# mschoenb97/po2_quantization

Hardware: AMD Instinct MI355X
Metric: quantized-conv fwd images/sec, ResNet56 224×224 bs=256; 1/2/4/8 MI355X (higher is better)
Workload: dtype fp32(bf16x3); 1 GPU; resnet56 quantized-conv chain: 56 fused po2-4bit quantize+conv fwd + head (stage-1 and stage-2 conv1->conv2 pairs as one launch each) (stride-2 conv1 + 1x1 shortcut of stages 2-3 as one launch each) (weight packs of the single-conv layers batched: one launch per 36); conv_pairs=True, conv_pairs_stage2=True, s2ds=True, pack_batch=True, autotune=True, image=224, batch_per_gpu=256, global_batch=256, quantizer=po2, bits=4, precision=bf16x3, parallelism=dp1, world_size=1, hip_graph=False

## Files before the change

### po2_quantization_amd/csrc/po2q_conv_pair64.hip

```cpp
#include <hip/hip_runtime.h>

#include <algorithm>
#include <climits>
#include <cstdint>
#include <cstdlib>
#include <map>
#include <mutex>
#include <string>
#include <type_traits>
#include <utility>

#include "../../include/po2q.h"
#include "po2q_internal.h"
#include "po2q_rows_dev.h"
#include "po2q_x3_dev.h"

namespace po2q {

namespace {
constexpr int kP6C = 64;
constexpr int kP6Wp = 64;
constexpr int kP6PL = (kP6Wp + 2) * 2 * kP6C;
constexpr int kP6Set = 3 * kP6PL;
constexpr int kP6Raw = kP6C * kP6Wp * 4;
constexpr int kP6RPB = kP6Wp * 4;
constexpr int kP6PD = 2;
constexpr int kP6KS = 6;
constexpr int kP6Lds = kP6PD * kP6Raw + 2 * kP6Set + 2 * kP6Set;
constexpr int kP6PackBytes = 3 * kP6KS * 4 * 64 * 16;

__device__ __forceinline__ int p6_addr(int P, int oc) { return P * 128 + ((oc ^ (P & 7)) << 4); }
}

struct Pair64Args {
    int N, H, W;
    int RB, nseg, items, remap;
    const uint4* wp1;
    const uint4* wp2;
    const float* s1;
    const float* s2;
    const float* b1;
    const float* b2;
};

template <int NG, int NTS>
__global__ __launch_bounds__(512, 1) void conv_pair64(const float* __restrict__ x, float* __restrict__ y,
                                                      Pair64Args a) {
    static_assert(NG == 3 || NG == 4, "column groups");
    constexpr int C = kP6C, KS = kP6KS, PL = kP6PL, SET = kP6Set, RPB = kP6RPB;
    extern __shared__ __attribute__((aligned(16))) unsigned char lds[];
    const int tid = threadIdx.x, lane = tid & 63;
    const int wave = __builtin_amdgcn_readfirstlane(tid >> 6);
    const bool roleA = wave >= 4;
    const int t = wave & 3;
    unsigned char* raw = lds;
    unsigned char* xp = raw + kP6PD * kP6Raw;

    int blk = blockIdx.x;
    if (a.remap) blk = (blk & 7) * (int)(gridDim.x >> 3) + (blk >> 3);
    if (blk >= a.items) return;
    const int seg = blk % a.nseg;
    const int n = blk / a.nseg;
    const int p0 = seg * a.RB;
    const int rbe = min(a.RB, a.H - p0);
    const int nx = rbe + 4;
    const int n1 = rbe + 2;
    const int nsteps = nx + 2;
    const int HW = a.H * a.W;
// ... 10 lines not shown
    float bk[4];
    {
        const float* b = roleA ? a.b2 : a.b1;
#pragma unroll
        for (int e = 0; e < 4; ++e) bk[e] = b ? b[roleA ? 16 * t + (lane & 15) : 16 * t + 4 * (lane >> 4) + e] : 0.0f;
    }
#pragma unroll
    for (int r = 0; r < 3; ++r)
#pragma unroll
        for (int ks = 0; ks < KS; ++ks) asm volatile("s_waitcnt vmcnt(0)" : "+v"(bw[r][ks]));
    asm volatile("s_waitcnt vmcnt(0)" : "+v"(scale), "+v"(bk[0]), "+v"(bk[1]), "+v"(bk[2]), "+v"(bk[3]));

    for (int e = tid; e < (4 * SET) / 16; e += 512) reinterpret_cast<uint4*>(xp)[e] = make_uint4(0u, 0u, 0u, 0u);
    __syncthreads();

    const __amdgpu_buffer_rsrc_t rs = rows_rsrc(x + (int64_t)n * C * HW, C * HW * 4);
    uint32_t vi[4];
#pragma unroll
    for (int i = 0; i < 4; ++i) {
        const int c = 16 * t + 4 * i + (lane >> 4), q = 4 * (lane & 15);
        vi[i] = q < a.W ? ((uint32_t)c * (uint32_t)HW + (uint32_t)q) * 4u : 0x7fffffffu;
    }
    const uint32_t raw_lds = (uint32_t)(uintptr_t)raw;
    auto load_x = [&](int sl, int jn) __attribute__((always_inline)) {
        const int h = p0 - 2 + jn;
        const bool hok = jn < nx && h >= 0 && h < a.H;
        const uint32_t roff = (uint32_t)(hok ? h : 0) * (uint32_t)a.W * 4u;
        const uint32_t base = raw_lds + (uint32_t)(sl * kP6Raw) + (uint32_t)(16 * t) * (uint32_t)RPB;
#pragma unroll
        for (int i = 0; i < 4; ++i)
            rows_dma16<(NTS & 2) != 0>(rs, (hok && vi[i] != 0x7fffffffu) ? vi[i] + roff : 0x7fffffffu, 0u,
                                       base + (uint32_t)i * 1024u);
    };
    int xwb[2] = {p6_addr(lane + 1, 2 * t) + kP6PD * kP6Raw, p6_addr(lane + 1, 2 * t + 1) + kP6PD * kP6Raw};
    asm volatile("" : "+v"(xwb[0]), "+v"(xwb[1]));
    auto split_x = [&](const unsigned char* rw, int pb) __attribute__((always_inline)) {
#pragma unroll
        for (int o = 0; o < 2; ++o) {
            uint32_t b8[8];
#pragma unroll
            for (int e = 0; e < 8; ++e)
                b8[e] = *reinterpret_cast<const uint32_t*>(rw + (16 * t + 8 * o + e) * RPB + lane * 4);
            uint4 hi, mid, lo;
            split3(b8, hi, mid, lo);
            unsigned char* pw = lds + (xwb[o] + pb);
            *reinterpret_cast<uint4*>(pw) = hi;
            *reinterpret_cast<uint4*>(pw + PL) = mid;
            *reinterpret_cast<uint4*>(pw + 2 * PL) = lo;
        }
    };

    int foff[KS];
    {
        const int p = lane & 15, g = lane >> 4;
        const int region = kP6PD * kP6Raw + (roleA ? 2 * SET : 0);
#pragma unroll
        for (int ks = 0; ks < KS; ++ks) {
            foff[ks] = p6_addr(p + ks % 3, 4 * (ks / 3) + g) + region;
            asm volatile("" : "+v"(foff[ks]));
        }
    }
    int ywb = p6_addr((lane & 15) + 1, 2 * t + (lane >> 5)) + 8 * ((lane >> 4) & 1) + kP6PD * kP6Raw + 2 * SET;
    asm volatile("" : "+v"(ywb));

    floatx4 acc[3][NG];
#pragma unroll
    for (int sl = 0; sl < 3; ++sl)
#pragma unroll
        for (int grp = 0; grp < NG; ++grp) acc[sl][grp] = floatx4{0.f, 0.f, 0.f, 0.f};

    auto mfmas = [&](auto S_, auto TR_, int pb) __attribute__((always_inline)) {
// ... 3 lines not shown
        bf16x8 af[2][NG];
        auto ldf = [&](bf16x8 (&f)[NG], int st) __attribute__((always_inline)) {
#pragma unroll
            for (int grp = 0; grp < NG; ++grp)
                f[grp] = __builtin_bit_cast(
                    bf16x8, *reinterpret_cast<const uint4*>(lds + (foff[st / 3] + (pb + (st % 3) * PL + grp * (16 * 128)))));
        };
        ldf(af[0], 0);
#pragma unroll
        for (int st = 0; st < 3 * KS; ++st) {
            if (st + 1 < 3 * KS) ldf(af[(st + 1) & 1], st + 1);
            const int ks = st / 3;
#pragma unroll
            for (int rr = 0; rr < 3; ++rr)
#pragma unroll
                for (int grp = 0; grp < NG; ++grp)
                    acc[SL[rr]][grp] =
                        TR ? __builtin_amdgcn_mfma_f32_16x16x32_bf16(bw[rr][ks], af[st & 1][grp], acc[SL[rr]][grp], 0, 0, 0)
                           : __builtin_amdgcn_mfma_f32_16x16x32_bf16(af[st & 1][grp], bw[rr][ks], acc[SL[rr]][grp], 0, 0, 0);
            __builtin_amdgcn_sched_barrier(0);
        }
    };

    floatx4 pend[NG];
#pragma unroll
    for (int grp = 0; grp < NG; ++grp) pend[grp] = floatx4{0.f, 0.f, 0.f, 0.f};

    auto stepB = [&](auto S_, int j) __attribute__((always_inline)) {
        constexpr int S6 = decltype(S_)::value;
        constexpr int S = S6 % 3;
        constexpr int D = (S + 2) % 3;
        constexpr int B2 = S6 & 1;
        asm volatile("s_waitcnt lgkmcnt(0)\n\ts_barrier" ::: "memory");
        load_x(B2, j + 2);
        {
            const int i1 = j - 3;
            const int r1 = p0 - 1 + i1;
            const bool irow = i1 >= 0 && i1 < n1 && r1 >= 0 && r1 < a.H;
            const int p = lane & 15;
            unsigned char* yw = lds + (ywb + (1 - B2) * SET);
#pragma unroll
            for (int grp = 0; grp < NG; ++grp) {
                const int q = 16 * grp + p;
                const bool okq = irow && q < a.W;
                uint32_t b4[4];
#pragma unroll
                for (int e = 0; e < 4; ++e) {
                    const float v = pend[grp][e] * scale + bk[e];
                    b4[e] = okq ? __float_as_uint(v) : 0u;
                }
                uint2 h2, m2, l2;
                split4p(b4, h2, m2, l2);
                unsigned char* yg = yw + grp * (16 * 128);
                *reinterpret_cast<uint2*>(yg) = h2;
                *reinterpret_cast<uint2*>(yg + PL) = m2;
                *reinterpret_cast<uint2*>(yg + 2 * PL) = l2;
            }
        }
        rows_wait<4>();
        split_x(raw + (1 - B2) * kP6Raw, (1 - B2) * SET);
        {
            const int h = p0 - 2 + j;
            if (j < nx && h >= 0 && h < a.H) mfmas(std::integral_constant<int, S>{}, std::true_type{}, B2 * SET);
        }
#pragma unroll
        for (int grp = 0; grp < NG; ++grp) {
            pend[grp] = acc[D][grp];
            acc[D][grp] = floatx4{0.f, 0.f, 0.f, 0.f};
        }
    };

    const __amdgpu_buffer_rsrc_t ry = rows_rsrc(y + (int64_t)n * C * HW, C * HW * 4);

    auto stepA = [&](auto S_, int j) __attribute__((always_inline)) {
        constexpr int S6 = decltype(S_)::value;
        constexpr int S = S6 % 3;
        constexpr int D = (S + 2) % 3;
        constexpr int YR = S6 & 1;
        asm volatile("s_waitcnt lgkmcnt(0)\n\ts_barrier" ::: "memory");
        {
            const int i2 = j - 4, r2 = p0 - 1 + i2;
            if (i2 >= 0 && i2 < n1 && r2 >= 0 && r2 < a.H)
                mfmas(std::integral_constant<int, S>{}, std::false_type{}, YR * SET);
        }
        const int o = j - 6;
        const bool orow = o >= 0 && o < rbe;
// ... 71 lines not shown

hipError_t pair64_launch(const float* x, float* y, int64_t N, int64_t H, int64_t W, const uint16_t* packed1,
                         const float* scale1, const uint16_t* packed2, const float* scale2, const float* bias1,
                         const float* bias2, hipStream_t s) {
    if (!pair64_geom_ok(N, kP6C, H, W)) return hipErrorInvalidValue;
    int64_t nseg = std::max<int64_t>(1, (256 + N - 1) / N);
    nseg = std::min<int64_t>(nseg, std::max<int64_t>(1, H / 8));
    if (const char* e = getenv("PO2Q_PAIR64_NSEG")) nseg = std::min<int64_t>(std::max(1, atoi(e)), H);
    Pair64Args a;
    a.N = (int)N; a.H = (int)H; a.W = (int)W;
    a.RB = (int)((H + nseg - 1) / nseg);
    a.nseg = (int)((H + a.RB - 1) / a.RB);
    const int64_t items = N * a.nseg;
    if (items > INT_MAX / 2) return hipErrorInvalidValue;
    const int blocks = (int)((items + 7) / 8 * 8);
    a.items = (int)items;
    a.remap = 1;
    a.wp1 = reinterpret_cast<const uint4*>(packed1);
    a.wp2 = reinterpret_cast<const uint4*>(packed2);
    a.s1 = scale1; a.s2 = scale2;
    a.b1 = bias1; a.b2 = bias2;
    int nts = 0;
    if (const char* e = getenv("PO2Q_PAIR64_NTS")) nts = atoi(e) == 0 ? 0 : 3;
    const dim3 grid((unsigned)blocks), block(512);
#define PO2Q_P6(g, t)                                                                            \
    if ((W <= 48 ? 3 : 4) == g && nts == t) {                                                    \
        hipLaunchKernelGGL((conv_pair64<g, t>), grid, block, (size_t)kP6Lds, s, x, y, a);        \
        return hipGetLastError();                                                                \
    }
    PO2Q_P6(4, 3) PO2Q_P6(3, 3) PO2Q_P6(4, 0) PO2Q_P6(3, 0)
#undef PO2Q_P6
    return hipErrorInvalidValue;
}

ConvPlan pair64_pack_plan(int64_t N, int64_t H, int64_t W) {
    ConvPlan p{};
    p.N = (int)N; p.C = kP6C; p.H = (int)H; p.W = (int)W; p.K = kP6C;
    p.R = p.S = 3; p.sh = p.sw = 1; p.ph = p.pw = 1; p.dh = p.dw = 1; p.groups = 1;
    p.P = p.H; p.Q = p.W; p.Cg = p.C; p.Kg = p.K;
    p.kind = KIND_BF16X3_ROWS;
    p.vrx = 1;
    p.CC = 32;
    p.nchunks = 2;
    p.steps = kP6KS;
    p.NT = 4;
    p.taps = 9;
    p.packed_floats = kP6PackBytes / 4;
    return p;
}

namespace {
constexpr size_t kP6Scratch = 256 + 2 * ((kP6PackBytes + 255) / 256 * 256);
char* pair64_scratch(hipStream_t s) {
// ... 77 lines not shown
```

### po2_quantization_amd/csrc/po2q_conv_pairw.hip

```cpp
#include <hip/hip_runtime.h>

#include <algorithm>
#include <climits>
#include <cstdint>
#include <cstdlib>
#include <string>
#include <type_traits>
#include <utility>

#include "../../include/po2q.h"
#include "po2q_epi.h"
#include "po2q_internal.h"
#include "po2q_quant_dev.h"
#include "po2q_rows_dev.h"
#include "po2q_x3_dev.h"

namespace po2q {

namespace {
constexpr int kPWC = 32;
constexpr int kPWSW = 32;
constexpr int kPWWaves = 4;
constexpr int kPWWp = kPWSW * kPWWaves;
constexpr int kPWPL = (kPWSW + 2) * 2 * kPWC + 32;
// ... 4 lines not shown

__device__ __forceinline__ int pw_oct(int P, int oc) { return P * 64 + 16 * (oc ^ ((P >> 1) & 3)); }

template <class F, int... R>
__device__ __forceinline__ void pw_unroll(F& f, std::integer_sequence<int, R...>) {
    (f(std::integral_constant<int, R>{}), ...);
}
}

struct PairWArgs {
    int N, H, W;
    int RB, nseg, items, remap;
    WQuant q1, q2;
    const float* b1;
    const float* b2;
    const float* ps1;
    const float* pb1;
    const float* ps2;
    const float* pb2;
    int act1, act2;
    const float* res;
};

template <int PD, int NTS, bool RES, int E, int DBG = 0>
__global__ __launch_bounds__(512, 1) void conv_pairw(const float* __restrict__ x, float* __restrict__ y,
                                                     PairWArgs a) {
    static_assert(PD >= 2 && PD <= 5, "raw ring slots");
    constexpr int CC = kPWC, SW = kPWSW, WC = SW + 2, PL = kPWPL, YPL = kPWYPL, RPB = kPWRPB;
    constexpr int NG = SW / 16, NT = CC / 16, KS = 3, NF = 3 * KS * NT;
    constexpr int yslot = 3 * YPL;
    extern __shared__ __attribute__((aligned(16))) unsigned char lds[];
    const int tid = threadIdx.x, lane = tid & 63;
    const int wave = __builtin_amdgcn_readfirstlane(tid >> 6);
    const bool roleA = wave >= kPWWaves;
    const int sw = wave & (kPWWaves - 1);
    unsigned char* raw = lds;
    unsigned char* yr = raw + PD * kPWRaw;
    unsigned char* slab = yr + 2 * yslot + sw * (3 * PL);
    unsigned char* resr = yr + 2 * yslot + kPWWaves * 3 * PL + sw * (PD * kPWRes);

    int blk = blockIdx.x;
    if (a.remap) blk = (blk & 7) * (int)(gridDim.x >> 3) + (blk >> 3);
    if (blk >= a.items) return;
    const int seg = blk % a.nseg;
    const int n = blk / a.nseg;
    const int p0 = seg * a.RB;
    const int rbe = min(a.RB, a.H - p0);
    const int nx = rbe + 4;
    const int n1 = rbe + 2;
    const int nsteps = nx + 2;
    const int q0 = sw * SW;
    const int HW = a.H * a.W;

    const __amdgpu_buffer_rsrc_t rs = rows_rsrc(x + (int64_t)n * CC * HW, CC * HW * 4);
    uint32_t vi[4];
#pragma unroll
    for (int i = 0; i < 4; ++i) {
        const int e = 64 * (4 * sw + i) + lane;
        const int c = e >> 5, q = 4 * (e & 31);
        vi[i] = q < a.W ? ((uint32_t)c * (uint32_t)HW + (uint32_t)q) * 4u : 0x7fffffffu;
    }
    const uint32_t raw_lds = (uint32_t)(uintptr_t)raw;
// ... 26 lines not shown
                              res_lds + (uint32_t)(sl * kPWRes) + i * 1024u);
    };

    const int cp = lane & 15, so = lane >> 4;
    const int rdx0 = (so * 8) * RPB + (q0 + 2 * cp) * 4;
    const int wa0 = pw_oct(2 * cp + 1, so), wa1 = pw_oct(2 * cp + 2, so);
    const int hl = lane & 31;
    const int hside = hl >> 4, hch = 16 * (lane >> 5) + (hl & 15);
    const int hq = hside ? q0 + SW : q0 - 1;
    const bool h_ok = hq >= 0 && hq < a.W;
    const int wa_h = pw_oct(hside ? WC - 1 : 0, hch >> 3) + (hch & 7) * 2;
    const int rdx_h = hch * RPB + (h_ok ? hq : 0) * 4;
    int foff[NG][KS];
    {
        const int p = lane & 15, g = lane >> 4;
#pragma unroll
        for (int grp = 0; grp < NG; ++grp)
#pragma unroll
            for (int ks = 0; ks < KS; ++ks) foff[grp][ks] = pw_oct((roleA ? q0 : 0) + 16 * grp + p + ks, g);
    }

    const __amdgpu_buffer_rsrc_t ry = rows_rsrc(y + (int64_t)n * CC * HW, CC * HW * 4);
    constexpr int ST = 2 * NT;
    constexpr int VMW_B = 4 * (PD - 2);
    constexpr int VMW_A = ST + (PD - 2) * (4 + ST);

    float scale = 1.0f;
    bool fin = true;
    bf16x8 bw[NF] = {};
    float bk[E ? NT * 4 : 1], es[E ? NT * 4 : 1], eb[E ? NT * 4 : 1];
    floatx4 acc[3][NG][NT];
#pragma unroll
    for (int sl = 0; sl < 3; ++sl)
#pragma unroll
        for (int grp = 0; grp < NG; ++grp)
#pragma unroll
            for (int nt = 0; nt < NT; ++nt) acc[sl][grp][nt] = floatx4{0.f, 0.f, 0.f, 0.f};

    auto mfmas = [&](auto S_, auto TR_, const unsigned char* pb) __attribute__((always_inline)) {
        constexpr int SR = decltype(S_)::value;
        constexpr bool TR = decltype(TR_)::value;
        constexpr int SL[3] = {(SR + 1) % 3, SR, (SR + 2) % 3};
        constexpr int PLS = TR ? PL : YPL;
        bf16x8 af[3][NG];
#pragma unroll
        for (int pl = 0; pl < 3; ++pl)
#pragma unroll
// ... 15 lines not shown
                        acc[SL[rr]][grp][nt] = TR ? __builtin_amdgcn_mfma_f32_16x16x32_bf16(b, af[pl][grp], c, 0, 0, 0)
                                                  : __builtin_amdgcn_mfma_f32_16x16x32_bf16(af[pl][grp], b, c, 0, 0, 0);
                    }
                    if (ks + 1 < KS)
                        af[pl][grp] = __builtin_bit_cast(
                            bf16x8, *reinterpret_cast<const uint4*>(pb + pl * PLS + foff[grp][ks + 1 < KS ? ks + 1 : 0]));
                }
    };

    auto zero_slot = [&](auto S_) __attribute__((always_inline)) {
        constexpr int SR = decltype(S_)::value;
#pragma unroll
        for (int grp = 0; grp < NG; ++grp)
#pragma unroll
            for (int nt = 0; nt < NT; ++nt) acc[(SR + 1) % 3][grp][nt] = floatx4{0.f, 0.f, 0.f, 0.f};
    };

    floatx4 pend[NG][NT];
#pragma unroll
    for (int grp = 0; grp < NG; ++grp)
#pragma unroll
        for (int nt = 0; nt < NT; ++nt) pend[grp][nt] = floatx4{0.f, 0.f, 0.f, 0.f};

    auto stepB = [&](auto S_, int j) __attribute__((always_inline)) {
        constexpr int S6 = decltype(S_)::value;
        constexpr int S = S6 % 3;
        constexpr int D = (S + 2) % 3;
        constexpr int YW = (S6 + 1) & 1;
        const int RS = (6 % PD == 0) ? S6 % PD : j % PD;
        if constexpr ((DBG & 32) != 0) {
            if constexpr (S6 % 2 == 0) rows_wait<0>();
        } else {
            rows_wait<VMW_B>();
        }
        if constexpr ((DBG & 16) == 0) asm volatile("s_waitcnt lgkmcnt(0)\n\ts_barrier" ::: "memory");
        if constexpr ((DBG & 32) != 0) {
            if constexpr (S6 % 2 == 0) {
                const int h = p0 + j;
                const bool hok = h + 1 < a.H;
                const uint32_t roff = (uint32_t)(hok ? h : 0) * (uint32_t)a.W * 4u;
                const uint32_t base = raw_lds + (uint32_t)((S6 / 2 % 2) * kPWRaw) + (uint32_t)(4 * sw) * 1024u;
#pragma unroll
                for (int i = 0; i < 8; ++i) {
                    const int e = 64 * (8 * sw + i) + lane;
                    const int c = e / 56, q = 4 * (e - c * 56);
                    const uint32_t vo = (hok && c < CC) ? ((uint32_t)c * (uint32_t)HW + (uint32_t)q) * 4u + roff : 0x7fffffffu;
                    rows_dma16<(NTS & 2) != 0>(rs, vo, 0u, base + (uint32_t)(i & 3) * 1024u);
                }
            }
        } else if constexpr ((DBG & 2) == 0) {
            load_x((6 % PD == 0) ? (S6 + PD - 1) % PD : (j - 1 + PD) % PD, j - 1 + PD);
        }
        uint32_t bx[2][8], hx;
        {
            const unsigned char* rw = raw + RS * kPWRaw;
#pragma unroll
            for (int e = 0; e < 8; ++e) {
                const uint2 v2 = *reinterpret_cast<const uint2*>(rw + rdx0 + e * RPB);
                bx[0][e] = v2.x;
                bx[1][e] = v2.y;
            }
            hx = *reinterpret_cast<const uint32_t*>(rw + rdx_h);
        }
        if constexpr ((DBG & 8) == 0) {
            const int i1 = j - 3;
            const int r1 = p0 - 1 + i1;
            const bool irow = i1 >= 0 && i1 < n1 && r1 >= 0 && r1 < a.H;
            const int p = lane & 15, g = lane >> 4;
            unsigned char* yw = yr + YW * yslot;
#pragma unroll
            for (int grp = 0; grp < NG; ++grp) {
                const int q = q0 + 16 * grp + p;
                const bool okq = irow && q < a.W;
#pragma unroll
                for (int nt = 0; nt < NT; ++nt) {
                    uint32_t b4[4];
#pragma unroll
                    for (int e = 0; e < 4; ++e) {
                        float t;
                        if constexpr (E == 0) {
                            t = pend[grp][nt][e] * scale + 0.0f;
                        } else if constexpr (E == 2) {
                            const int c = nt * 4 + e;
                            t = pend[grp][nt][e] * es[c] + eb[c];
                            t = t < 0.0f ? 0.0f : t;
                        } else {
                            const int c = nt * 4 + e;
                            t = epi_act((pend[grp][nt][e] * scale + bk[c]) * es[c] + eb[c], a.act1);
                        }
                        b4[e] = okq ? __float_as_uint(t) : 0u;
                    }
                    uint2 h2, m2, l2;
                    split4p<false>(b4, h2, m2, l2);
                    const int wo = pw_oct(q + 1, (4 * nt + g) >> 1) + 8 * (g & 1);
                    *reinterpret_cast<uint2*>(yw + wo) = h2;
                    *reinterpret_cast<uint2*>(yw + YPL + wo) = m2;
                    *reinterpret_cast<uint2*>(yw + 2 * YPL + wo) = l2;
                }
            }
        }
        if constexpr ((DBG & 8) == 0) {
            uint4 hi, mid, lo;
            split3<false>(bx[0], hi, mid, lo);
            *reinterpret_cast<uint4*>(slab + wa0) = hi;
            *reinterpret_cast<uint4*>(slab + PL + wa0) = mid;
            *reinterpret_cast<uint4*>(slab + 2 * PL + wa0) = lo;
            split3<false>(bx[1], hi, mid, lo);
            *reinterpret_cast<uint4*>(slab + wa1) = hi;
            *reinterpret_cast<uint4*>(slab + PL + wa1) = mid;
            *reinterpret_cast<uint4*>(slab + 2 * PL + wa1) = lo;
            uint16_t h16, m16, l16;
            split1(h_ok ? hx : 0u, h16, m16, l16);
            *reinterpret_cast<uint16_t*>(slab + wa_h) = h16;
            *reinterpret_cast<uint16_t*>(slab + PL + wa_h) = m16;
            *reinterpret_cast<uint16_t*>(slab + 2 * PL + wa_h) = l16;
        }
        if constexpr ((DBG & 1) == 0) {
            const int h = p0 - 2 + j;
            if (j < nx && h >= 0 && h < a.H)
                mfmas(std::integral_constant<int, S>{}, std::true_type{}, slab);
            else
                zero_slot(std::integral_constant<int, S>{});
        }
#pragma unroll
        for (int grp = 0; grp < NG; ++grp)
#pragma unroll
            for (int nt = 0; nt < NT; ++nt) pend[grp][nt] = acc[D][grp][nt];
    };

    auto stepA = [&](auto S_, int j) __attribute__((always_inline)) {
        constexpr int S6 = decltype(S_)::value;
        constexpr int S = S6 % 3;
        constexpr int D = (S + 2) % 3;
        constexpr int YR = S6 & 1;
        const int RS = (6 % PD == 0) ? S6 % PD : j % PD;
        if constexpr (RES) rows_wait<VMW_A>();
        if constexpr ((DBG & 16) == 0) asm volatile("s_waitcnt lgkmcnt(0)\n\ts_barrier" ::: "memory");
        if constexpr (RES) load_res((6 % PD == 0) ? (S6 + PD - 1) % PD : (j - 1 + PD) % PD, j - 1 + PD);
// ... 43 lines not shown
                sa[e] = __int_as_float(__builtin_amdgcn_update_dpp(__float_as_int(vv[0][e]), __float_as_int(vv[1][e]),
                                                                   0x128, 0xf, 0xc, false));
                sb[e] = __int_as_float(__builtin_amdgcn_update_dpp(__float_as_int(vv[1][e]), __float_as_int(vv[0][e]),
                                                                   0x128, 0xf, 0x3, false));
            }
            const uint32_t ca = (uint32_t)(16 * nt) + (uint32_t)(lane & 7), cb = ca + 8u;
            if constexpr ((DBG & 32) != 0) {
                if constexpr (S6 % 2 == 1) {
                    const uint32_t ro2 = rowoff >= (uint32_t)a.W ? rowoff - (uint32_t)a.W : rowoff;
                    rows_store<(NTS & 1) != 0>(ry, ok ? (ca * (uint32_t)HW + ro2) * 4u : 0x7fffffffu, sa);
                    rows_store<(NTS & 1) != 0>(ry, ok ? (ca * (uint32_t)HW + rowoff) * 4u : 0x7fffffffu, sa);
                    rows_store<(NTS & 1) != 0>(ry, ok ? (cb * (uint32_t)HW + ro2) * 4u : 0x7fffffffu, sb);
                    rows_store<(NTS & 1) != 0>(ry, ok ? (cb * (uint32_t)HW + rowoff) * 4u : 0x7fffffffu, sb);
                }
            } else if constexpr ((DBG & 4) == 0) {
                rows_store<(NTS & 1) != 0>(ry, ok ? (ca * (uint32_t)HW + rowoff) * 4u : 0x7fffffffu, sa);
                rows_store<(NTS & 1) != 0>(ry, ok ? (cb * (uint32_t)HW + rowoff) * 4u : 0x7fffffffu, sb);
            }
        }
    };

    if (!roleA) {
#pragma unroll
        for (int r = 0; r < PD - 1; ++r) load_x(r, r);
    } else if constexpr (RES) {
        const floatx4 z = floatx4{0.f, 0.f, 0.f, 0.f};
#pragma unroll
        for (int r = 0; r < PD - 1; ++r) {
            load_res(r, r);
#pragma unroll
            for (int i = 0; i < ST; ++i) rows_store<(NTS & 1) != 0>(ry, 0x7fffffffu, z);
        }
    }
    {
        unsigned* red = reinterpret_cast<unsigned*>(yr);
        unsigned* thr = red + 16;
        uint4* fr = reinterpret_cast<uint4*>(yr + 4096);
        static_assert(4096 + 2 * NF * 64 * 16 <= 2 * yslot, "fragment scratch");
        bool fin1, fin2;
        const float scale1 = wq_prologue(a.q1, thr, red, 2 * kPWWaves, fin1);
        if constexpr ((DBG & 128) == 0) wq_pack_rows_lds<CC>(a.q1, CC, CC, NT, KS, scale1, fin1, thr, fr, NF);
        const float scale2 = wq_prologue(a.q2, thr, red, 2 * kPWWaves, fin2);
        if constexpr ((DBG & 128) == 0) {
            wq_pack_rows_lds<CC>(a.q2, CC, CC, NT, KS, scale2, fin2, thr, fr + NF * 64, NF);
            const uint4* frw = fr + (roleA ? NF * 64 : 0);
#pragma unroll
            for (int f = 0; f < NF; ++f) bw[f] = __builtin_bit_cast(bf16x8, frw[f * 64 + lane]);
// ... 19 lines not shown
        }
#pragma unroll
        for (int f = 0; f < NF; ++f) asm volatile("" : "+v"(bw[f]));
        if constexpr (E == 2) {
#pragma unroll
            for (int c = 0; c < NT * 4; ++c) {
                eb[c] = bk[c] * es[c] + eb[c];
                es[c] = scale * es[c];
            }
        }
        if constexpr (E != 0) {
            if (roleA) {
#pragma unroll
                for (int nt = 0; nt < NT; ++nt) {
                    bk[nt] = bk[nt * 4];
                    es[nt] = es[nt * 4];
                    eb[nt] = eb[nt * 4];
                }
            }
        }
        __syncthreads();
        for (int e = tid; e < (2 * yslot) / 16; e += blockDim.x)
            reinterpret_cast<uint4*>(yr)[e] = make_uint4(0u, 0u, 0u, 0u);
    }
    (void)fin;
    if constexpr ((DBG & 64) != 0) return;
    if (roleA) {
        for (int j = 0; j < nsteps; j += 6) {
            stepA(std::integral_constant<int, 0>{}, j);
            stepA(std::integral_constant<int, 1>{}, j + 1);
            stepA(std::integral_constant<int, 2>{}, j + 2);
            if (j + 3 >= nsteps) break;
            stepA(std::integral_constant<int, 3>{}, j + 3);
            stepA(std::integral_constant<int, 4>{}, j + 4);
            stepA(std::integral_constant<int, 5>{}, j + 5);
        }
    } else {
        for (int j = 0; j < nsteps; j += 6) {
            stepB(std::integral_constant<int, 0>{}, j);
            stepB(std::integral_constant<int, 1>{}, j + 1);
            stepB(std::integral_constant<int, 2>{}, j + 2);
            if (j + 3 >= nsteps) break;
            stepB(std::integral_constant<int, 3>{}, j + 3);
            stepB(std::integral_constant<int, 4>{}, j + 4);
            stepB(std::integral_constant<int, 5>{}, j + 5);
        }
    }
    asm volatile("s_waitcnt vmcnt(0)" ::: "memory");
}

namespace {

size_t pairw_lds(int pd, bool res) {
    return (size_t)pd * kPWRaw + 2 * 3 * (size_t)kPWYPL + (size_t)kPWWaves * 3 * kPWPL +
           (res ? (size_t)kPWWaves * pd * kPWRes : 0);
}

template <int PD, int NTS>
hipError_t launch_pairw_t(int blocks, size_t lds, const PairWArgs& a, const float* x, float* y, bool res, hipStream_t s) {
    const bool plain = !res && !a.b1 && !a.b2 && !a.ps1 && !a.pb1 && !a.ps2 && !a.pb2 && a.act1 == 0 && a.act2 == 0;
    const dim3 grid((unsigned)blocks), block(64 * 2 * kPWWaves);
#ifdef PO2Q_PAIRW_DIAG
    if (const char* dv = getenv("PO2Q_PAIR_W32_DBG")) {
        const int dbg = atoi(dv);
#define PO2Q_PWD(v) \
        if (dbg == v && plain && NTS == 3) { \
            hipLaunchKernelGGL((conv_pairw<PD, NTS, false, 0, v>), grid, block, lds, s, x, y, a); \
            return hipGetLastError(); \
        }
        PO2Q_PWD(9) PO2Q_PWD(11) PO2Q_PWD(13) PO2Q_PWD(15) PO2Q_PWD(25) PO2Q_PWD(29) PO2Q_PWD(27)
        PO2Q_PWD(31) PO2Q_PWD(64) PO2Q_PWD(192) PO2Q_PWD(128)
#undef PO2Q_PWD
    }
#endif
    if (plain) {
        hipLaunchKernelGGL((conv_pairw<PD, NTS, false, 0>), grid, block, lds, s, x, y, a);
        return hipGetLastError();
    }
    if constexpr (PD == 2) {
        if (res && a.act1 == 1 && a.act2 == 1)
            hipLaunchKernelGGL((conv_pairw<PD, NTS, true, 2>), grid, block, lds, s, x, y, a);
        else if (res)
            hipLaunchKernelGGL((conv_pairw<PD, NTS, true, 1>), grid, block, lds, s, x, y, a);
        else
            hipLaunchKernelGGL((conv_pairw<PD, NTS, false, 1>), grid, block, lds, s, x, y, a);
        return hipGetLastError();
    }
    return hipErrorInvalidValue;
}

int pairw_knob() {
    const char* e = getenv("PO2Q_PAIR_W32");
    return (e && e[0] == '0') ? 0 : 1;
}

}

bool pairw_applicable(int64_t N, int64_t C, int64_t H, int64_t W) {
    return C == 32 && W > 3 * kPWSW && W <= kPWWp && W % 4 == 0 && N > 0 && H > 0 && pairw_knob() != 0 &&
           (int64_t)C * H * W * 4 < (1LL << 31);
}

hipError_t pairw_launch(const float* x, const float* w1, const float* w2, float* y, int64_t N, int64_t H,
                        int64_t W, int bits, int fsr, int mode, const float* bias1, const float* bias2,
                        const float* post_scale1, const float* post_shift1, int act1, const float* post_scale2,
                        const float* post_shift2, const float* residual, int act2, hipStream_t s) {
    const bool res = residual != nullptr;
    const int pd = 2;
    int nts = res ? 1 : 3;
    if (const char* e = getenv("PO2Q_PAIR_W32_NTS")) nts = atoi(e) == 1 ? 1 : 3;
    const size_t lds = pairw_lds(pd, res);
    if (lds > 160 * 1024) return hipErrorInvalidValue;
    int nseg = std::max<int64_t>(1, (256 + N - 1) / N);
    nseg = std::min<int>(nseg, std::max<int>(1, (int)H / 8));
    PairWArgs a;
    a.N = (int)N; a.H = (int)H; a.W = (int)W;
    a.RB = (int)((H + nseg - 1) / nseg);
    a.nseg = (int)((H + a.RB - 1) / a.RB);
    const int64_t items = N * a.nseg;
    if (items > INT_MAX / 2) return hipErrorInvalidValue;
    const int blocks = (int)((items + 7) / 8 * 8);
    a.items = (int)items;
    a.remap = (blocks % 8 == 0) ? 1 : 0;
    const int lo = fsr - (1 << (bits - 1)), hi = fsr - 1;
    a.q1.w = w1; a.q1.n = 32 * 32 * 9; a.q1.lo = lo; a.q1.hi = hi; a.q1.mode = mode - 1;
    a.q2 = a.q1;
    a.q2.w = w2;
    a.b1 = bias1; a.b2 = bias2;
    a.ps1 = post_scale1; a.pb1 = post_shift1; a.act1 = act1;
    a.ps2 = post_scale2; a.pb2 = post_shift2; a.act2 = act2;
    a.res = residual;
#define PO2Q_PW(d, t) \
    if (pd == d && nts == t) return launch_pairw_t<d, t>(blocks, lds, a, x, y, res, s);
    PO2Q_PW(2, 3)
#ifndef PO2Q_PAIRW_ISA
    PO2Q_PW(2, 1)
#endif
#undef PO2Q_PW
    return hipErrorInvalidValue;
}

}
```

Before: 26580 images/s.

## Interleave input DMA, epilogue and split work into MFMA stream for conv pairs

Adds a PIPE variant of the pair64 and pairw conv-pair kernels. It spreads the row DMA issue, the conv1 epilogue split writes and the raw-to-bf16x3 split of the next row between MFMA groups, instead of running them serially before the MFMAs. The pairw variant double-buffers the split slab so the next row can be prepared while the current one is consumed. The pipelined path is on by default, except for residual pairw launches. It costs more LDS, larger unrolled code and more register pressure, and the hand-placed sched_barriers could hurt scheduling.

```diff
diff --git a/po2_quantization_amd/csrc/po2q_conv_pair64.hip b/po2_quantization_amd/csrc/po2q_conv_pair64.hip
--- a/po2_quantization_amd/csrc/po2q_conv_pair64.hip
+++ b/po2_quantization_amd/csrc/po2q_conv_pair64.hip
@@ -30,6 +30,11 @@
 constexpr int kP6PackBytes = 3 * kP6KS * 4 * 64 * 16;
 
 __device__ __forceinline__ int p6_addr(int P, int oc) { return P * 128 + ((oc ^ (P & 7)) << 4); }
+
+template <class F, int... R>
+__device__ __forceinline__ void p6_unroll(F&& f, std::integer_sequence<int, R...>) {
+    (f(std::integral_constant<int, R>{}), ...);
+}
 }
 
 struct Pair64Args {
@@ -43,7 +48,7 @@
     const float* b2;
 };
 
-template <int NG, int NTS>
+template <int NG, int NTS, bool PIPE>
 __global__ __launch_bounds__(512, 1) void conv_pair64(const float* __restrict__ x, float* __restrict__ y,
                                                       Pair64Args a) {
     static_assert(NG == 3 || NG == 4, "column groups");
@@ -100,31 +105,39 @@
         vi[i] = q < a.W ? ((uint32_t)c * (uint32_t)HW + (uint32_t)q) * 4u : 0x7fffffffu;
     }
     const uint32_t raw_lds = (uint32_t)(uintptr_t)raw;
-    auto load_x = [&](int sl, int jn) __attribute__((always_inline)) {
+    auto load_x1 = [&](int sl, int jn, int i) __attribute__((always_inline)) {
         const int h = p0 - 2 + jn;
         const bool hok = jn < nx && h >= 0 && h < a.H;
         const uint32_t roff = (uint32_t)(hok ? h : 0) * (uint32_t)a.W * 4u;
         const uint32_t base = raw_lds + (uint32_t)(sl * kP6Raw) + (uint32_t)(16 * t) * (uint32_t)RPB;
-#pragma unroll
-        for (int i = 0; i < 4; ++i)
-            rows_dma16<(NTS & 2) != 0>(rs, (hok && vi[i] != 0x7fffffffu) ? vi[i] + roff : 0x7fffffffu, 0u,
-                                       base + (uint32_t)i * 1024u);
+        rows_dma16<(NTS & 2) != 0>(rs, (hok && vi[i] != 0x7fffffffu) ? vi[i] + roff : 0x7fffffffu, 0u,
+                                   base + (uint32_t)i * 1024u);
+    };
+    auto load_x = [&](int sl, int jn) __attribute__((always_inline)) {
+#pragma unroll
+        for (int i = 0; i < 4; ++i) load_x1(sl, jn, i);
     };
     int xwb[2] = {p6_addr(lane + 1, 2 * t) + kP6PD * kP6Raw, p6_addr(lane + 1, 2 * t + 1) + kP6PD * kP6Raw};
     asm volatile("" : "+v"(xwb[0]), "+v"(xwb[1]));
+    auto split_rd = [&](const unsigned char* rw, int o, uint32_t (&b8)[8]) __attribute__((always_inline)) {
+#pragma unroll
+        for (int e = 0; e < 8; ++e)
+            b8[e] = *reinterpret_cast<const uint32_t*>(rw + (16 * t + 8 * o + e) * RPB + lane * 4);
+    };
+    auto split_wr = [&](int o, int pb, const uint32_t (&b8)[8]) __attribute__((always_inline)) {
+        uint4 hi, mid, lo;
+        split3(b8, hi, mid, lo);
+        unsigned char* pw = lds + (xwb[o] + pb);
+        *reinterpret_cast<uint4*>(pw) = hi;
+        *reinterpret_cast<uint4*>(pw + PL) = mid;
+        *reinterpret_cast<uint4*>(pw + 2 * PL) = lo;
+    };
     auto split_x = [&](const unsigned char* rw, int pb) __attribute__((always_inline)) {
 #pragma unroll
         for (int o = 0; o < 2; ++o) {
             uint32_t b8[8];
-#pragma unroll
-            for (int e = 0; e < 8; ++e)
-                b8[e] = *reinterpret_cast<const uint32_t*>(rw + (16 * t + 8 * o + e) * RPB + lane * 4);
-            uint4 hi, mid, lo;
-            split3(b8, hi, mid, lo);
-            unsigned char* pw = lds + (xwb[o] + pb);
-            *reinterpret_cast<uint4*>(pw) = hi;
-            *reinterpret_cast<uint4*>(pw + PL) = mid;
-            *reinterpret_cast<uint4*>(pw + 2 * PL) = lo;
+            split_rd(rw, o, b8);
+            split_wr(o, pb, b8);
         }
     };
 
@@ -174,6 +187,37 @@
         }
     };
 
+    auto mfmas_pipe = [&](auto S_, int pb, auto&& pre, auto&& hook) __attribute__((always_inline)) {
+        constexpr int S = decltype(S_)::value;
+        constexpr int SL[3] = {(S + 1) % 3, S, (S + 2) % 3};
+        bf16x8 af[2][NG];
+        auto ldf = [&](bf16x8 (&f)[NG], int st) __attribute__((always_inline)) {
+#pragma unroll
+            for (int grp = 0; grp < NG; ++grp)
+                f[grp] = __builtin_bit_cast(
+                    bf16x8, *reinterpret_cast<const uint4*>(lds + (foff[st / 3] + (pb + (st % 3) * PL + grp * (16 * 128)))));
+        };
+        ldf(af[0], 0);
+        auto stage = [&](auto ST_) __attribute__((always_inline)) {
+            constexpr int st = decltype(ST_)::value;
+            constexpr int ks = st / 3;
+            pre(ST_);
+            if constexpr (st + 1 < 3 * KS) ldf(af[(st + 1) & 1], st + 1);
+            __builtin_amdgcn_sched_barrier(0);
+            auto row = [&](auto RR_) __attribute__((always_inline)) {
+                constexpr int rr = decltype(RR_)::value;
+#pragma unroll
+                for (int grp = 0; grp < NG; ++grp)
+                    acc[SL[rr]][grp] =
+                        __builtin_amdgcn_mfma_f32_16x16x32_bf16(bw[rr][ks], af[st & 1][grp], acc[SL[rr]][grp], 0, 0, 0);
+                hook(std::integral_constant<int, 3 * st + rr>{});
+                __builtin_amdgcn_sched_barrier(0);
+            };
+            p6_unroll(row, std::make_integer_sequence<int, 3>{});
+        };
+        p6_unroll(stage, std::make_integer_sequence<int, 3 * KS>{});
+    };
+
     floatx4 pend[NG];
 #pragma unroll
     for (int grp = 0; grp < NG; ++grp) pend[grp] = floatx4{0.f, 0.f, 0.f, 0.f};
@@ -184,36 +228,60 @@
         constexpr int D = (S + 2) % 3;
         constexpr int B2 = S6 & 1;
         asm volatile("s_waitcnt lgkmcnt(0)\n\ts_barrier" ::: "memory");
-        load_x(B2, j + 2);
-        {
-            const int i1 = j - 3;
-            const int r1 = p0 - 1 + i1;
-            const bool irow = i1 >= 0 && i1 < n1 && r1 >= 0 && r1 < a.H;
-            const int p = lane & 15;
-            unsigned char* yw = lds + (ywb + (1 - B2) * SET);
-#pragma unroll
-            for (int grp = 0; grp < NG; ++grp) {
-                const int q = 16 * grp + p;
-                const bool okq = irow && q < a.W;
-                uint32_t b4[4];
-#pragma unroll
-                for (int e = 0; e < 4; ++e) {
-                    const float v = pend[grp][e] * scale + bk[e];
-                    b4[e] = okq ? __float_as_uint(v) : 0u;
+        const int i1 = j - 3;
+        const int r1 = p0 - 1 + i1;
+        const bool irow = i1 >= 0 && i1 < n1 && r1 >= 0 && r1 < a.H;
+        unsigned char* yw = lds + (ywb + (1 - B2) * SET);
+        auto epi1 = [&](int grp) __attribute__((always_inline)) {
+            const int q = 16 * grp + (lane & 15);
+            const bool okq = irow && q < a.W;
+            uint32_t b4[4];
+#pragma unroll
+            for (int e = 0; e < 4; ++e) {
+                const float v = pend[grp][e] * scale + bk[e];
+                b4[e] = okq ? __float_as_uint(v) : 0u;
+            }
+            uint2 h2, m2, l2;
+            split4p(b4, h2, m2, l2);
+            unsigned char* yg = yw + grp * (16 * 128);
+            *reinterpret_cast<uint2*>(yg) = h2;
+            *reinterpret_cast<uint2*>(yg + PL) = m2;
+            *reinterpret_cast<uint2*>(yg + 2 * PL) = l2;
+        };
+        const int hx = p0 - 2 + j;
+        const bool xrow = j < nx && hx >= 0 && hx < a.H;
+        if constexpr (!PIPE) {
+            load_x(B2, j + 2);
+#pragma unroll
+            for (int grp = 0; grp < NG; ++grp) epi1(grp);
+            rows_wait<4>();
+            split_x(raw + (1 - B2) * kP6Raw, (1 - B2) * SET);
+            if (xrow) mfmas(std::integral_constant<int, S>{}, std::true_type{}, B2 * SET);
+        } else {
+            uint32_t b8[8];
+            const unsigned char* rw = raw + (1 - B2) * kP6Raw;
+            auto pre = [&](auto ST_) __attribute__((always_inline)) {
+                constexpr int st = decltype(ST_)::value;
+                if constexpr (st < 4) load_x1(B2, j + 2, st);
+            };
+            auto hook = [&](auto K_) __attribute__((always_inline)) {
+                constexpr int K = decltype(K_)::value;
+                if constexpr (K % 2 == 1 && K / 2 < NG) epi1(K / 2);
+                if constexpr (K == 10) {
+                    rows_wait<4>();
+                    split_rd(rw, 0, b8);
                 }
-                uint2 h2, m2, l2;
-                split4p(b4, h2, m2, l2);
-                unsigned char* yg = yw + grp * (16 * 128);
-                *reinterpret_cast<uint2*>(yg) = h2;
-                *reinterpret_cast<uint2*>(yg + PL) = m2;
-                *reinterpret_cast<uint2*>(yg + 2 * PL) = l2;
+                if constexpr (K == 12) split_wr(0, (1 - B2) * SET, b8);
+                if constexpr (K == 13) split_rd(rw, 1, b8);
+                if constexpr (K == 15) split_wr(1, (1 - B2) * SET, b8);
+            };
+            static_assert(2 * (NG - 1) + 1 < 10, "epilogue-1 tiles come before the split");
+            if (xrow) {
+                mfmas_pipe(std::integral_constant<int, S>{}, B2 * SET, pre, hook);
+            } else {
+                p6_unroll(pre, std::make_integer_sequence<int, 4>{});
+                p6_unroll(hook, std::make_integer_sequence<int, 16>{});
             }
-        }
-        rows_wait<4>();
-        split_x(raw + (1 - B2) * kP6Raw, (1 - B2) * SET);
-        {
-            const int h = p0 - 2 + j;
-            if (j < nx && h >= 0 && h < a.H) mfmas(std::integral_constant<int, S>{}, std::true_type{}, B2 * SET);
         }
 #pragma unroll
         for (int grp = 0; grp < NG; ++grp) {
@@ -331,13 +399,16 @@
     a.b1 = bias1; a.b2 = bias2;
     int nts = 0;
     if (const char* e = getenv("PO2Q_PAIR64_NTS")) nts = atoi(e) == 0 ? 0 : 3;
+    bool pipe = true;
+    if (const char* e = getenv("PO2Q_PAIR64_PIPE")) pipe = e[0] != '0';
     const dim3 grid((unsigned)blocks), block(512);
-#define PO2Q_P6(g, t)                                                                            \
-    if ((W <= 48 ? 3 : 4) == g && nts == t) {                                                    \
-        hipLaunchKernelGGL((conv_pair64<g, t>), grid, block, (size_t)kP6Lds, s, x, y, a);        \
+#define PO2Q_P6(g, t, p)                                                                         \
+    if ((W <= 48 ? 3 : 4) == g && nts == t && pipe == p) {                                       \
+        hipLaunchKernelGGL((conv_pair64<g, t, p>), grid, block, (size_t)kP6Lds, s, x, y, a);     \
         return hipGetLastError();                                                                \
     }
-    PO2Q_P6(4, 3) PO2Q_P6(3, 3) PO2Q_P6(4, 0) PO2Q_P6(3, 0)
+    PO2Q_P6(4, 0, true) PO2Q_P6(3, 0, true) PO2Q_P6(4, 3, true) PO2Q_P6(3, 3, true)
+    PO2Q_P6(4, 0, false) PO2Q_P6(3, 0, false) PO2Q_P6(4, 3, false) PO2Q_P6(3, 3, false)
 #undef PO2Q_P6
     return hipErrorInvalidValue;
 }
diff --git a/po2_quantization_amd/csrc/po2q_conv_pairw.hip b/po2_quantization_amd/csrc/po2q_conv_pairw.hip
--- a/po2_quantization_amd/csrc/po2q_conv_pairw.hip
+++ b/po2_quantization_amd/csrc/po2q_conv_pairw.hip
@@ -50,10 +50,12 @@
     const float* res;
 };
 
-template <int PD, int NTS, bool RES, int E, int DBG = 0>
+template <int PD, int NTS, bool RES, int E, bool PIPE, int DBG = 0>
 __global__ __launch_bounds__(512, 1) void conv_pairw(const float* __restrict__ x, float* __restrict__ y,
                                                      PairWArgs a) {
     static_assert(PD >= 2 && PD <= 5, "raw ring slots");
+    static_assert(!PIPE || (PD == 2 && !RES && DBG == 0), "the pipelined schedule: 2 raw slots, no residual");
+    constexpr int NSET = PIPE ? 2 : 1;
     constexpr int CC = kPWC, SW = kPWSW, WC = SW + 2, PL = kPWPL, YPL = kPWYPL, RPB = kPWRPB;
     constexpr int NG = SW / 16, NT = CC / 16, KS = 3, NF = 3 * KS * NT;
     constexpr int yslot = 3 * YPL;
@@ -64,8 +66,8 @@
     const int sw = wave & (kPWWaves - 1);
     unsigned char* raw = lds;
     unsigned char* yr = raw + PD * kPWRaw;
-    unsigned char* slab = yr + 2 * yslot + sw * (3 * PL);
-    unsigned char* resr = yr + 2 * yslot + kPWWaves * 3 * PL + sw * (PD * kPWRes);
+    unsigned char* slab = yr + 2 * yslot + sw * (NSET * 3 * PL);
+    unsigned char* resr = yr + 2 * yslot + kPWWaves * NSET * 3 * PL + sw * (PD * kPWRes);
 
     int blk = blockIdx.x;
     if (a.remap) blk = (blk & 7) * (int)(gridDim.x >> 3) + (blk >> 3);
@@ -138,7 +140,7 @@
 
     const __amdgpu_buffer_rsrc_t ry = rows_rsrc(y + (int64_t)n * CC * HW, CC * HW * 4);
     constexpr int ST = 2 * NT;
-    constexpr int VMW_B = 4 * (PD - 2);
+    constexpr int VMW_B = PIPE ? 0 : 4 * (PD - 2);
     constexpr int VMW_A = ST + (PD - 2) * (4 + ST);
 
     float scale = 1.0f;
@@ -200,6 +202,129 @@
 #pragma unroll
         for (int nt = 0; nt < NT; ++nt) pend[grp][nt] = floatx4{0.f, 0.f, 0.f, 0.f};
 
+    auto epi1 = [&](unsigned char* yw, bool irow, int grp, int nt) __attribute__((always_inline)) {
+        const int p = lane & 15, g = lane >> 4;
+        const int q = q0 + 16 * grp + p;
+        const bool okq = irow && q < a.W;
+        uint32_t b4[4];
+#pragma unroll
+        for (int e = 0; e < 4; ++e) {
+            float t;
+            if constexpr (E == 0) {
+                t = pend[grp][nt][e] * scale + 0.0f;
+            } else if constexpr (E == 2) {
+                const int c = nt * 4 + e;
+                t = pend[grp][nt][e] * es[c] + eb[c];
+                t = t < 0.0f ? 0.0f : t;
+            } else {
+                const int c = nt * 4 + e;
+                t = epi_act((pend[grp][nt][e] * scale + bk[c]) * es[c] + eb[c], a.act1);
+            }
+            b4[e] = okq ? __float_as_uint(t) : 0u;
+        }
+        uint2 h2, m2, l2;
+        split4p<false>(b4, h2, m2, l2);
+        const int wo = pw_oct(q + 1, (4 * nt + g) >> 1) + 8 * (g & 1);
+        *reinterpret_cast<uint2*>(yw + wo) = h2;
+        *reinterpret_cast<uint2*>(yw + YPL + wo) = m2;
+        *reinterpret_cast<uint2*>(yw + 2 * YPL + wo) = l2;
+    };
+    auto raw_rd = [&](const unsigned char* rw, uint32_t (&bx)[2][8], uint32_t& hx) __attribute__((always_inline)) {
+#pragma unroll
+        for (int e = 0; e < 8; ++e) {
+            const uint2 v2 = *reinterpret_cast<const uint2*>(rw + rdx0 + e * RPB);
+            bx[0][e] = v2.x;
+            bx[1][e] = v2.y;
+        }
+        hx = *reinterpret_cast<const uint32_t*>(rw + rdx_h);
+    };
+    auto split_half = [&](unsigned char* sp, int h, const uint32_t (&bx)[2][8]) __attribute__((always_inline)) {
+        const int wa = h ? wa1 : wa0;
+        uint4 hi, mid, lo;
+        split3<false>(bx[h], hi, mid, lo);
+        *reinterpret_cast<uint4*>(sp + wa) = hi;
+        *reinterpret_cast<uint4*>(sp + PL + wa) = mid;
+        *reinterpret_cast<uint4*>(sp + 2 * PL + wa) = lo;
+    };
+    auto split_halo = [&](unsigned char* sp, uint32_t hx) __attribute__((always_inline)) {
+        uint16_t h16, m16, l16;
+        split1(h_ok ? hx : 0u, h16, m16, l16);
+        *reinterpret_cast<uint16_t*>(sp + wa_h) = h16;
+        *reinterpret_cast<uint16_t*>(sp + PL + wa_h) = m16;
+        *reinterpret_cast<uint16_t*>(sp + 2 * PL + wa_h) = l16;
+    };
+
+    auto mfmas_pipe = [&](auto S_, const unsigned char* pb, auto&& hook) __attribute__((always_inline)) {
+        constexpr int SR = decltype(S_)::value;
+        constexpr int SL[3] = {(SR + 1) % 3, SR, (SR + 2) % 3};
+        bf16x8 af[3][NG];
+#pragma unroll
+        for (int pl = 0; pl < 3; ++pl)
+#pragma unroll
+            for (int grp = 0; grp < NG; ++grp)
+                af[pl][grp] = __builtin_bit_cast(bf16x8, *reinterpret_cast<const uint4*>(pb + pl * PL + foff[grp][0]));
+        auto unit = [&](auto U_) __attribute__((always_inline)) {
+            constexpr int u = decltype(U_)::value;
+            constexpr int ks = u / (3 * NG), pl = (u / NG) % 3, grp = u % NG;
+            __builtin_amdgcn_sched_barrier(0);
+#pragma unroll
+            for (int m = 0; m < 6; ++m) {
+                const int r3 = m / NT, nt = m % NT;
+                const int rr = 2 - r3;
+                const bf16x8 b = bw[(rr * KS + ks) * NT + nt];
+                const floatx4 c = (rr == 0 && ks == 0 && pl == 0) ? floatx4{0.f, 0.f, 0.f, 0.f} : acc[SL[rr]][grp][nt];
+                acc[SL[rr]][grp][nt] = __builtin_amdgcn_mfma_f32_16x16x32_bf16(b, af[pl][grp], c, 0, 0, 0);
+            }
+            hook(U_);
+            if constexpr (ks + 1 < KS)
+                af[pl][grp] = __builtin_bit_cast(
+                    bf16x8, *reinterpret_cast<const uint4*>(pb + pl * PL + foff[grp][ks + 1 < KS ? ks + 1 : 0]));
+        };
+        pw_unroll(unit, std::make_integer_sequence<int, 3 * KS * NG>{});
+        __builtin_amdgcn_sched_barrier(0);
+    };
+
+    auto stepBP = [&](auto S_, int j) __attribute__((always_inline)) {
+        constexpr int S6 = decltype(S_)::value;
+        constexpr int S = S6 % 3;
+        constexpr int D = (S + 2) % 3;
+        constexpr int YW = (S6 + 1) & 1;
+        constexpr int P = S6 & 1;
+        rows_wait<VMW_B>();
+        asm volatile("s_waitcnt lgkmcnt(0)\n\ts_barrier" ::: "memory");
+        load_x(P, j + 2);
+        const int i1 = j - 3;
+        const int r1 = p0 - 1 + i1;
+        const bool irow = i1 >= 0 && i1 < n1 && r1 >= 0 && r1 < a.H;
+        unsigned char* yw = yr + YW * yslot;
+        const unsigned char* rw = raw + (1 - P) * kPWRaw;
+        unsigned char* sp = slab + (1 - P) * (3 * PL);
+        uint32_t bx[2][8], hx;
+        auto hook = [&](auto U_) __attribute__((always_inline)) {
+            constexpr int u = decltype(U_)::value;
+            if constexpr (u == 0) epi1(yw, irow, 0, 0);
+            if constexpr (u == 1) raw_rd(rw, bx, hx);
+            if constexpr (u == 3) split_half(sp, 0, bx);
+            if constexpr (u == 4) split_half(sp, 1, bx);
+            if constexpr (u == 5) split_halo(sp, hx);
+            if constexpr (u == 7) epi1(yw, irow, 0, 1);
+            if constexpr (u == 9) epi1(yw, irow, 1, 0);
+            if constexpr (u == 11) epi1(yw, irow, 1, 1);
+        };
+        static_assert(NG == 2 && NT == 2, "the slice table");
+        const int h = p0 - 2 + j;
+        if (j < nx && h >= 0 && h < a.H) {
+            mfmas_pipe(std::integral_constant<int, S>{}, slab + P * (3 * PL), hook);
+        } else {
+            pw_unroll(hook, std::make_integer_sequence<int, 12>{});
+            zero_slot(std::integral_constant<int, S>{});
+        }
+#pragma unroll
+        for (int grp = 0; grp < NG; ++grp)
+#pragma unroll
+            for (int nt = 0; nt < NT; ++nt) pend[grp][nt] = acc[D][grp][nt];
+    };
+
     auto stepB = [&](auto S_, int j) __attribute__((always_inline)) {
         constexpr int S6 = decltype(S_)::value;
         constexpr int S = S6 % 3;
@@ -230,68 +355,21 @@
             load_x((6 % PD == 0) ? (S6 + PD - 1) % PD : (j - 1 + PD) % PD, j - 1 + PD);
         }
         uint32_t bx[2][8], hx;
-        {
-            const unsigned char* rw = raw + RS * kPWRaw;
-#pragma unroll
-            for (int e = 0; e < 8; ++e) {
-                const uint2 v2 = *reinterpret_cast<const uint2*>(rw + rdx0 + e * RPB);
-                bx[0][e] = v2.x;
-                bx[1][e] = v2.y;
-            }
-            hx = *reinterpret_cast<const uint32_t*>(rw + rdx_h);
-        }
+        raw_rd(raw + RS * kPWRaw, bx, hx);
         if constexpr ((DBG & 8) == 0) {
             const int i1 = j - 3;
             const int r1 = p0 - 1 + i1;
             const bool irow = i1 >= 0 && i1 < n1 && r1 >= 0 && r1 < a.H;
-            const int p = lane & 15, g = lane >> 4;
             unsigned char* yw = yr + YW * yslot;
 #pragma unroll
-            for (int grp = 0; grp < NG; ++grp) {
-                const int q = q0 + 16 * grp + p;
-                const bool okq = irow && q < a.W;
-#pragma unroll
-                for (int nt = 0; nt < NT; ++nt) {
-                    uint32_t b4[4];
-#pragma unroll
-                    for (int e = 0; e < 4; ++e) {
-                        float t;
-                        if constexpr (E == 0) {
-                            t = pend[grp][nt][e] * scale + 0.0f;
-                        } else if constexpr (E == 2) {
-                            const int c = nt * 4 + e;
-                            t = pend[grp][nt][e] * es[c] + eb[c];
-                            t = t < 0.0f ? 0.0f : t;
-                        } else {
-                            const int c = nt * 4 + e;
-                            t = epi_act((pend[grp][nt][e] * scale + bk[c]) * es[c] + eb[c], a.act1);
-                        }
-                        b4[e] = okq ? __float_as_uint(t) : 0u;
-                    }
-                    uint2 h2, m2, l2;
-                    split4p<false>(b4, h2, m2, l2);
-                    const int wo = pw_oct(q + 1, (4 * nt + g) >> 1) + 8 * (g & 1);
-                    *reinterpret_cast<uint2*>(yw + wo) = h2;
-                    *reinterpret_cast<uint2*>(yw + YPL + wo) = m2;
-                    *reinterpret_cast<uint2*>(yw + 2 * YPL + wo) = l2;
-                }
-            }
+            for (int grp = 0; grp < NG; ++grp)
+#pragma unroll
+                for (int nt = 0; nt < NT; ++nt) epi1(yw, irow, grp, nt);
         }
         if constexpr ((DBG & 8) == 0) {
-            uint4 hi, mid, lo;
-            split3<false>(bx[0], hi, mid, lo);
-            *reinterpret_cast<uint4*>(slab + wa0) = hi;
-            *reinterpret_cast<uint4*>(slab + PL + wa0) = mid;
-            *reinterpret_cast<uint4*>(slab + 2 * PL + wa0) = lo;
-            split3<false>(bx[1], hi, mid, lo);
-            *reinterpret_cast<uint4*>(slab + wa1) = hi;
-            *reinterpret_cast<uint4*>(slab + PL + wa1) = mid;
-            *reinterpret_cast<uint4*>(slab + 2 * PL + wa1) = lo;
-            uint16_t h16, m16, l16;
-            split1(h_ok ? hx : 0u, h16, m16, l16);
-            *reinterpret_cast<uint16_t*>(slab + wa_h) = h16;
-            *reinterpret_cast<uint16_t*>(slab + PL + wa_h) = m16;
-            *reinterpret_cast<uint16_t*>(slab + 2 * PL + wa_h) = l16;
+            split_half(slab, 0, bx);
+            split_half(slab, 1, bx);
+            split_halo(slab, hx);
         }
         if constexpr ((DBG & 1) == 0) {
             const int h = p0 - 2 + j;
@@ -381,7 +459,7 @@
 
     if (!roleA) {
 #pragma unroll
-        for (int r = 0; r < PD - 1; ++r) load_x(r, r);
+        for (int r = 0; r < (PIPE ? 2 : PD - 1); ++r) load_x(r, r);
     } else if constexpr (RES) {
         const floatx4 z = floatx4{0.f, 0.f, 0.f, 0.f};
 #pragma unroll
@@ -447,6 +525,15 @@
         __syncthreads();
         for (int e = tid; e < (2 * yslot) / 16; e += blockDim.x)
             reinterpret_cast<uint4*>(yr)[e] = make_uint4(0u, 0u, 0u, 0u);
+        if constexpr (PIPE) {
+            if (!roleA) {
+                uint32_t bx[2][8], hx;
+                raw_rd(raw, bx, hx);
+                split_half(slab, 0, bx);
+                split_half(slab, 1, bx);
+                split_halo(slab, hx);
+            }
+        }
     }
     (void)fin;
     if constexpr ((DBG & 64) != 0) return;
@@ -462,13 +549,16 @@
         }
     } else {
         for (int j = 0; j < nsteps; j += 6) {
-            stepB(std::integral_constant<int, 0>{}, j);
-            stepB(std::integral_constant<int, 1>{}, j + 1);
-            stepB(std::integral_constant<int, 2>{}, j + 2);
+            auto step = [&](auto S_, int jj) __attribute__((always_inline)) {
+                if constexpr (PIPE) stepBP(S_, jj); else stepB(S_, jj);
+            };
+            step(std::integral_constant<int, 0>{}, j);
+            step(std::integral_constant<int, 1>{}, j + 1);
+            step(std::integral_constant<int, 2>{}, j + 2);
             if (j + 3 >= nsteps) break;
-            stepB(std::integral_constant<int, 3>{}, j + 3);
-            stepB(std::integral_constant<int, 4>{}, j + 4);
-            stepB(std::integral_constant<int, 5>{}, j + 5);
+            step(std::integral_constant<int, 3>{}, j + 3);
+            step(std::integral_constant<int, 4>{}, j + 4);
+            step(std::integral_constant<int, 5>{}, j + 5);
         }
     }
     asm volatile("s_waitcnt vmcnt(0)" ::: "memory");
@@ -476,13 +566,14 @@
 
 namespace {
 
-size_t pairw_lds(int pd, bool res) {
-    return (size_t)pd * kPWRaw + 2 * 3 * (size_t)kPWYPL + (size_t)kPWWaves * 3 * kPWPL +
+size_t pairw_lds(int pd, bool res, bool pipe) {
+    return (size_t)pd * kPWRaw + 2 * 3 * (size_t)kPWYPL + (size_t)kPWWaves * (pipe ? 2 : 1) * 3 * kPWPL +
            (res ? (size_t)kPWWaves * pd * kPWRes : 0);
 }
 
 template <int PD, int NTS>
-hipError_t launch_pairw_t(int blocks, size_t lds, const PairWArgs& a, const float* x, float* y, bool res, hipStream_t s) {
+hipError_t launch_pairw_t(int blocks, size_t lds, const PairWArgs& a, const float* x, float* y, bool res, bool pipe,
+                          hipStream_t s) {
     const bool plain = !res && !a.b1 && !a.b2 && !a.ps1 && !a.pb1 && !a.ps2 && !a.pb2 && a.act1 == 0 && a.act2 == 0;
     const dim3 grid((unsigned)blocks), block(64 * 2 * kPWWaves);
 #ifdef PO2Q_PAIRW_DIAG
@@ -490,7 +581,7 @@
         const int dbg = atoi(dv);
 #define PO2Q_PWD(v) \
         if (dbg == v && plain && NTS == 3) { \
-            hipLaunchKernelGGL((conv_pairw<PD, NTS, false, 0, v>), grid, block, lds, s, x, y, a); \
+            hipLaunchKernelGGL((conv_pairw<PD, NTS, false, 0, false, v>), grid, block, lds, s, x, y, a); \
             return hipGetLastError(); \
         }
         PO2Q_PWD(9) PO2Q_PWD(11) PO2Q_PWD(13) PO2Q_PWD(15) PO2Q_PWD(25) PO2Q_PWD(29) PO2Q_PWD(27)
@@ -498,17 +589,19 @@
 #undef PO2Q_PWD
     }
 #endif
-    if (plain) {
-        hipLaunchKernelGGL((conv_pairw<PD, NTS, false, 0>), grid, block, lds, s, x, y, a);
-        return hipGetLastError();
-    }
     if constexpr (PD == 2) {
-        if (res && a.act1 == 1 && a.act2 == 1)
-            hipLaunchKernelGGL((conv_pairw<PD, NTS, true, 2>), grid, block, lds, s, x, y, a);
+        if (plain && pipe)
+            hipLaunchKernelGGL((conv_pairw<PD, NTS, false, 0, true>), grid, block, lds, s, x, y, a);
+        else if (plain)
+            hipLaunchKernelGGL((conv_pairw<PD, NTS, false, 0, false>), grid, block, lds, s, x, y, a);
+        else if (res && a.act1 == 1 && a.act2 == 1)
+            hipLaunchKernelGGL((conv_pairw<PD, NTS, true, 2, false>), grid, block, lds, s, x, y, a);
         else if (res)
-            hipLaunchKernelGGL((conv_pairw<PD, NTS, true, 1>), grid, block, lds, s, x, y, a);
+            hipLaunchKernelGGL((conv_pairw<PD, NTS, true, 1, false>), grid, block, lds, s, x, y, a);
+        else if (pipe)
+            hipLaunchKernelGGL((conv_pairw<PD, NTS, false, 1, true>), grid, block, lds, s, x, y, a);
         else
-            hipLaunchKernelGGL((conv_pairw<PD, NTS, false, 1>), grid, block, lds, s, x, y, a);
+            hipLaunchKernelGGL((conv_pairw<PD, NTS, false, 1, false>), grid, block, lds, s, x, y, a);
         return hipGetLastError();
     }
     return hipErrorInvalidValue;
@@ -534,7 +627,12 @@
     const int pd = 2;
     int nts = res ? 1 : 3;
     if (const char* e = getenv("PO2Q_PAIR_W32_NTS")) nts = atoi(e) == 1 ? 1 : 3;
-    const size_t lds = pairw_lds(pd, res);
+    bool pipe = !res;
+    if (const char* e = getenv("PO2Q_PAIR_W32_PIPE")) pipe = pipe && e[0] != '0';
+#ifdef PO2Q_PAIRW_DIAG
+    if (getenv("PO2Q_PAIR_W32_DBG")) pipe = false;
+#endif
+    const size_t lds = pairw_lds(pd, res, pipe);
     if (lds > 160 * 1024) return hipErrorInvalidValue;
     int nseg = std::max<int64_t>(1, (256 + N - 1) / N);
     nseg = std::min<int>(nseg, std::max<int>(1, (int)H / 8));
@@ -556,7 +654,7 @@
     a.ps2 = post_scale2; a.pb2 = post_shift2; a.act2 = act2;
     a.res = residual;
 #define PO2Q_PW(d, t) \
-    if (pd == d && nts == t) return launch_pairw_t<d, t>(blocks, lds, a, x, y, res, s);
+    if (pd == d && nts == t) return launch_pairw_t<d, t>(blocks, lds, a, x, y, res, pipe, s);
     PO2Q_PW(2, 3)
 #ifndef PO2Q_PAIRW_ISA
     PO2Q_PW(2, 1)
```

Result: faster. 26910 images/s, median of 6 (+1.2%).
